# AdamCodd/local-hyperDB

Hardware: AMD Instinct MI355X
Metric: queries/sec, N=10M d=384 fp16 top-100 (single-query stream; p50 latency alongside) (higher is better)
Workload: dtype f16; 1 GPU; N=10000000 d=384 fp16 Q=1 cosine_similarity top-100, row-sharded x1; rows_per_gpu=10000000, accumulate=f32, exchange=none

## Files before the change

### local-hyperdb_amd/csrc/hdb_api.hip

```cpp
#include "hdb_common.h"
#include "hdb_quant.h"
#include "hdb_ws.h"
#include "hdb_plan.h"
#include "../../include/hyperdb_hip.h"
#include <string>
#include <cmath>
#include <cstring>
#include <cstdio>
#include <algorithm>
#include <vector>
#include <chrono>
#include <atomic>

static thread_local std::string g_err;
static int fail(int code, const std::string& msg) { g_err = msg; return code; }
#define HIP_TRY(expr)                                                                              \
    do {                                                                                           \
        hipError_t e_ = (expr);                                                                    \
        if (e_ != hipSuccess)                                                                      \
            return fail(HDB_ERR_HIP, std::string(#expr) + ": " + hipGetErrorString(e_));           \
    } while (0)
#define LAUNCH_TRY(expr)                                                                           \
    do {                                                                                           \
        int e_ = (expr);                                                                           \
// ... 638 lines not shown
    if (ix->n == 0) return HDB_OK;
    HIP_TRY(hipSetDevice(ix->device));
    hipStream_t st = (hipStream_t)stream;
    const int W = (ix->d + 31) / 32;
    ScoresWs w;
    int rc = ws_lay(ix, w, ix->d, W);
    if (rc) return rc;
    float* qinv = w.qinv; float* qsq = w.qsq; int* qnan = w.qnan; uint32_t* qbits = w.qbits; void* qc = w.qc;
    LAUNCH_TRY(hdb_launch_qprep(dev_q, 1, ix->d, ix->dtype == HDB_F64, qinv, qsq, qnan, nullptr, nullptr, st));
    if (is_bits_metric(metric)) {
        rc = ensure_bits(ix, st); if (rc) return rc;
        LAUNCH_TRY(hdb_launch_qsign(dev_q, 1, ix->d, ix->dtype == HDB_F64, W, qbits, st));
    }
    ScanArgs a; base_args(ix, a, dev_q, metric);
    if (metric == HDB_PEARSON) {
        rc = ensure_pscale(ix, st); if (rc) return rc;
        LAUNCH_TRY(hdb_launch_qcentre(dev_q, 1, ix->d, ix->dtype == HDB_F64, qc, qinv, st));
        a.Q = qc; a.metric = HDB_COSINE; a.inv_norm = ix->pscale;
    }
    a.mask = nullptr;
    a.raw = 1;
    a.scores = dev_out; a.ld = ix->n;
    QueryBufs qb{qinv, qsq, qbits, nullptr, nullptr};
    return run_scan(ix, a, 0, 1, qb, false, false, st);
}

struct TopkArgs { const void* Q; int32_t nq, k; int metric; int64_t* idx; float* score; int32_t* status; hipStream_t st; };
static TopkFacts topk_facts(const hdb_index* ix) {
    return {ix->n, ix->d, ix->dtype, ix->qmode, ix->qauto, ix->qauto_declined, ix->pnib != nullptr, ix->plane_declined,
            ix->mask != nullptr, ix->bias != nullptr, hdb_cu_count(), ix->subset_m};
}

static int quant_pitch(const hdb_index* ix) { return (int)align_up((size_t)ix->d, 16); }
static size_t quant_ws_bytes(const hdb_index* ix, int nq, uint32_t pl_cap, bool mflavour) {
    return ws_bytes_for<QuantWs>(nq, quant_pitch(ix), (int)ix->d, quant_ld_max(ix->n, ix->d), pl_cap, mflavour);
}
static int quant_ws_lay(hdb_index* ix, QuantWs& w, int nq, uint32_t pl_cap, bool mflavour) {
    return ws_lay(ix, w, nq, quant_pitch(ix), (int)ix->d, quant_ld_max(ix->n, ix->d), pl_cap, mflavour);
}
static size_t quant_batch_ws_bytes(const hdb_index* ix, int cq) {
    return ws_bytes_for<QuantBatchWs>(cq, quant_pitch(ix), (int)ix->d, quant_batch_sample(ix->n).ld_s, quant_batch_wld());
}
static int quant_batch_ws_lay(hdb_index* ix, QuantBatchWs& w, int cq) {
    return ws_lay(ix, w, cq, quant_pitch(ix), (int)ix->d, quant_batch_sample(ix->n).ld_s, quant_batch_wld());
}
static void quant_base_args(const hdb_index* ix, QuantArgs& a, const int8_t* qcodes, const float* qaux, const float* qinv, int metric, int nq) {
    memset(&a, 0, sizeof(a));
    a.codes = ix->qcodes; a.n = ix->n; a.d = ix->d; a.P = ix->qP; a.aux = ix->qaux; a.sqnorm = ix->sqnorm; a.inv_norm = ix->inv_norm;
    a.qcodes = qcodes; a.qaux = qaux; a.qinv = qinv; a.bias = ix->bias; a.mask = ix->mask; a.metric = metric; a.nq = nq;
    a.gamma = (float)quant_gamma(ix->d);
}
static int quant_query_prep(hdb_index* ix, const float* Q, int nq, const QuantWs& w, bool mflavour, int* stat, uint32_t* cnt_init,
                            uint32_t* pl_cnt, hipStream_t st) {
    if (mflavour) {
        LAUNCH_TRY(hdb_launch_quant_qprep_m(Q, nq, ix->d, ix->qP, w.qinv, w.qsq, w.qnan, w.q16, w.qscl, w.qcodes, w.qaux, stat, cnt_init, pl_cnt, st));
    } else {
        LAUNCH_TRY(hdb_launch_qprep(Q, nq, ix->d, false, w.qinv, w.qsq, w.qnan, nullptr, nullptr, st));
        LAUNCH_TRY(hdb_launch_quant_qprep(Q, nq, ix->d, ix->qP, w.qcodes, w.qaux, stat, pl_cnt, st));
    }
    return HDB_OK;
}

static int shadow_prepare(hdb_index* ix, const TopkPlan& p, int nq, hipStream_t st, bool* declined) {
    if (p.build_needed) {
        const size_t ws_need = p.path == HDB_PATH_QUANT ? quant_ws_bytes(ix, nq, 0, true) : quant_batch_ws_bytes(ix, p.cq_max);
        if (!quant_auto_build(ix, ws_need, st)) { *declined = true; return HDB_OK; }
    }
    if (p.plane_wanted && !ix->pnib) {
        const int rc = plane_rows(ix, 0, ix->n, st);
        if (rc) return rc;
        *declined = ix->pnib == nullptr;
    }
    return HDB_OK;
}

static int quant_topk(hdb_index* ix, const TopkArgs& c, const TopkPlan& p) {
    const void* dev_Q = c.Q; const int32_t nq = c.nq, k = c.k; const int metric = c.metric; hipStream_t st = c.st;
    int64_t* dev_idx = c.idx; float* dev_score = c.score; int32_t* dev_status = c.status;
    const uint32_t kk = p.kk; const bool mflavour = p.mflavour, use_pl = p.plane_wanted;
    const int64_t n = ix->n;
    const uint32_t m = 16;
    const QuantSample sp = p.qs;
    QuantWs w;
    int rc = quant_ws_lay(ix, w, nq, 0, mflavour);
    if (rc) return rc;
    uint32_t* qstat = reinterpret_cast<uint32_t*>(ix->qstat);
    uint32_t* pl_cnt = use_pl ? qstat + 1 : nullptr;
    const size_t crow = (size_t)nq * HDB_CAND_CAP;
    const int nsub = p.nsub;
    rc = quant_query_prep(ix, (const float*)dev_Q, nq, w, mflavour, ix->qstat, nsub ? w.cnt : nullptr, pl_cnt, st);
    if (rc) return rc;
    QuantArgs a; quant_base_args(ix, a, w.qcodes, w.qaux, w.qinv, metric, nq);
    a.ntiles = sp.s_tiles; a.tile_stride = sp.s_stride; a.scores = w.sbuf; a.ld = sp.ld_s;
    a.wmax = w.wmax; a.nsub = nsub; a.thr_out = w.thr;
    LAUNCH_TRY(hdb_launch_quant_scan(&a, 0, (int)ix->opt.max_blocks, st));
    if (!nsub) LAUNCH_TRY(hdb_launch_sample_thr(w.sbuf, sp.s_rows, sp.ld_s, nq, m, w.thr, w.cnt, nullptr, st));
    a.ntiles = (n + 15) / 16; a.tile_stride = 1; a.scores = nullptr; a.ld = 0;
    a.thr = w.thr; a.cnt = w.cnt; a.cand = w.cand; a.cap = HDB_CAND_CAP;
    const bool has_bias = ix->bias != nullptr || ix->mask != nullptr;
    if (mflavour) {
        a.V = (const char*)ix->V; a.row_bytes = ix->d * 2; a.G = w.G;
        a.ginv = metric == HDB_COSINE ? w.ginv : nullptr; a.gbias = has_bias ? w.gbias : nullptr;
    }
    prof_begin(ix, st);
    if (use_pl) {
        a.pl_nib = ix->pnib; a.pl_bit = ix->pbit; a.pl_rec = ix->prec; a.pl_units = ix->pU;
        a.pl_cnt = pl_cnt; a.pl_cap = p.pl_cap;
        LAUNCH_TRY(hdb_launch_quant_plane_scan(&a, 0, (int)ix->opt.max_blocks, st));
    } else {
        LAUNCH_TRY(hdb_launch_quant_scan(&a, 1, (int)ix->opt.max_blocks, st));
    }
    prof_end(ix, st);
    if (mflavour) {
        ScanArgs s; memset(&s, 0, sizeof(s));
        s.V = w.G; s.n = (int64_t)crow; s.d = ix->d; s.Q = dev_Q; s.metric = metric; s.inv_norm = w.ginv; s.qinv = w.qinv;
        s.bias = has_bias ? w.gbias : nullptr; s.mask = nullptr; s.nq = nq;
        s.tile_stride = 1; s.ntiles = (int64_t)crow / hdb_mfma_tile_rows(ix->dtype, ix->d); s.cap = HDB_CAND_CAP;
        s.scores = w.gsc; s.ld = (int64_t)crow;
        LAUNCH_TRY(hdb_launch_mfma_scan(&s, ix->dtype, 0, nq, w.q16, w.ginv, w.qsq, w.qscl, (int)ix->opt.max_blocks, (int)ix->opt.mfma_variant, st, nullptr));
    } else {
        LAUNCH_TRY(hdb_launch_quant_rescore(ix->V, ix->d, ix->dtype, (const float*)dev_Q, nq, metric, ix->inv_norm, w.qinv, ix->bias, ix->mask,
                                            w.cand, w.cnt, HDB_CAND_CAP, st));
    }
    LAUNCH_TRY(hdb_launch_quant_finalize(w.cand, w.cnt, HDB_CAND_CAP, nq, (uint32_t)k, kk, ix->row_base, dev_idx, dev_score, dev_status, w.qnan,
                                         w.qaux, w.thr, ix->qstat, mflavour ? w.cand : nullptr, w.gsc, (int64_t)crow, st));
    return HDB_OK;
}

extern "C" int hdb_debug_quant_bounds(hdb_index* ix, const float* dev_q, int metric, float* dev_hi, float* dev_hi5, void* stream) {
    if (!ix || !dev_q || !dev_hi || !dev_hi5) return fail(HDB_ERR_ARG, "hdb_debug_quant_bounds: null argument");
    if (metric != HDB_DOT && metric != HDB_COSINE) return fail(HDB_ERR_ARG, "hdb_debug_quant_bounds: dot or cosine");
    if (ix->qmode != HDB_QUANT_I8 || !ix->pnib || ix->n < 1) return fail(HDB_ERR_UNSUPPORTED, "hdb_debug_quant_bounds: the index has no 5-bit plane");
    HIP_TRY(hipSetDevice(ix->device));
    hipStream_t st = (hipStream_t)stream;
    QuantWs w;
    int rc = quant_ws_lay(ix, w, 1, 0, true);
    if (rc) return rc;
    rc = quant_query_prep(ix, dev_q, 1, w, ix->qauto, nullptr, nullptr, nullptr, st);
    if (rc) return rc;
    QuantArgs a; quant_base_args(ix, a, w.qcodes, w.qaux, w.qinv, metric, 1);
    a.ntiles = (ix->n + 15) / 16; a.tile_stride = 1;
    a.pl_nib = ix->pnib; a.pl_bit = ix->pbit; a.pl_rec = ix->prec; a.pl_units = ix->pU;
    a.dbg = dev_hi;
    LAUNCH_TRY(hdb_launch_quant_scan_one(&a, 2, (int)ix->opt.max_blocks, st));
    a.dbg = dev_hi5;
    LAUNCH_TRY(hdb_launch_quant_plane_scan(&a, 1, (int)ix->opt.max_blocks, st));
    return HDB_OK;
}

static int quant_batch_topk(hdb_index* ix, const TopkArgs& c, const TopkPlan& p) {
    const void* dev_Q = c.Q; const int32_t nq = c.nq, k = c.k; const int metric = c.metric; hipStream_t st = c.st;
    int64_t* dev_idx = c.idx; float* dev_score = c.score; int32_t* dev_status = c.status;
    const uint32_t kk = p.kk;
    const int64_t n = ix->n;
    const int P = ix->qP;
    const uint32_t m = HDB_QB_SAMPLE_M;
    const QuantSample sp = p.qs;
    const int64_t s_tiles = sp.s_tiles, s_stride = sp.s_stride, s_rows = sp.s_rows, ld_s = sp.ld_s;
    const int cq_max = p.cq_max;
    QuantBatchWs w;
    const int rc = quant_batch_ws_lay(ix, w, cq_max);
    if (rc) return rc;
    const int64_t wld = quant_batch_wld();
    float* const qinv = w.qinv; float* const qsq = w.qsq; int* const qnan = w.qnan; float* const qscl = w.qscl;
    int8_t* const qcodes = w.qcodes; float* const qaux = w.qaux; float* const thr = w.thr; uint32_t* const cnt = w.cnt;
    unsigned long long* const cand = w.cand; void* const q16 = w.q16; float* const wbuf = w.wbuf;
    for (int q0 = 0; q0 < nq; q0 += cq_max) {
        const int cq = std::min(cq_max, nq - q0);
        const float* Qc = (const float*)dev_Q + (size_t)q0 * ix->d;
// ... 673 lines not shown
```

### local-hyperdb_amd/csrc/hdb_caps.h

```cpp
#pragma once
#include "../../include/hyperdb_hip.h"

static inline int hdb_scan_auto_blocks(int dtype, int row_bytes, bool vec, bool wide_rows) {
    if (dtype == HDB_F8E4M3 && vec && (row_bytes == 256 || row_bytes == 384 || row_bytes == 512)) {
        const int b = 512 * 768 / row_bytes;
        return b < 1024 ? b : 1024;
    }
    return wide_rows ? 256 : 512;
}

#define HDB_KS_MAX_SLICES 8
struct KsGeom {
    int slices;
    int width[HDB_KS_MAX_SLICES];
    int off[HDB_KS_MAX_SLICES];
};
static inline KsGeom ks_list(int elem_bytes, int n0, int w0, int n1 = 0, int w1 = 0) {
    KsGeom g = {};
    int at = 0;
    for (int s = 0; s < n0 + n1 && s < HDB_KS_MAX_SLICES; ++s) {
        g.width[s] = s < n0 ? w0 : w1; g.off[s] = at * elem_bytes;
        at += g.width[s];
    }
    g.slices = n0 + n1;
// ... 127 lines not shown
static inline int hdb_mfma_fused_blocks(int64_t ntiles, int cus, int max_blocks) {
    int blocks = (int)(ntiles < cus ? ntiles : cus);
    if (max_blocks > 0 && max_blocks < blocks) blocks = max_blocks;
    if (blocks > HDB_FUSED_MAX_WG) blocks = HDB_FUSED_MAX_WG;
    if (blocks < 1) blocks = 1;
    return blocks;
}

#ifndef HDB_BITS_THREADS
#define HDB_BITS_THREADS 1024
#endif
#define HDB_BITS_MAXW 512
static inline int hdb_bits_fused_supported(int metric, int nq, int W, uint32_t kk) {
    return (metric == HDB_HAMMING || metric == HDB_JACCARD) && nq >= 1 && nq <= 4 && W <= HDB_BITS_MAXW && kk <= 128;
}
static inline int hdb_bits_fused_blocks(int64_t ntiles, int cus, int max_blocks) {
    int blocks = cus;
    const int64_t items = ntiles * 4;
    if ((int64_t)blocks * HDB_BITS_THREADS > items) blocks = (int)((items + HDB_BITS_THREADS - 1) / HDB_BITS_THREADS);
    if (max_blocks > 0 && max_blocks < blocks) blocks = max_blocks;
    if (blocks < 1) blocks = 1;
    return blocks;
}
static inline bool hdb_bits_fused_local(int blocks, uint32_t kk) { return (int64_t)blocks >= 2 * (int64_t)kk; }

static inline int hdb_l1_tile_supported(int dtype, int d) {
    if (dtype == HDB_F16) return d == 128 || d == 256 || d == 384 || d == 512 || d == 640 || d == 768;
    if (dtype == HDB_F32) return d == 128 || d == 256 || d == 384 || d == 512 || d == 768;
    return 0;
}

static inline int hdb_quant_scan_blocks(int64_t ntiles, int max_blocks) { return hdb_grid_for(ntiles, 4, max_blocks > 0 ? max_blocks : 1024); }
static inline int hdb_quant_plane_units(int P) { return (P + 31) / 32; }

static inline int hdb_qb_supported(int d) { return d == 128 || d == 256 || d == 384 || d == 512; }
static inline void qb_shape(int nq, int& wq, int& nqt) {
    const int tq = (nq + 15) / 16;
    wq = tq <= 4 ? 1 : tq <= 8 ? 2 : 4;
    nqt = (tq + wq - 1) / wq;
}
static inline int hdb_qb_scan_blocks(int64_t ntiles, int nq, int cus, int max_blocks) {
    int wq, nqt; qb_shape(nq, wq, nqt);
    const int64_t lim = max_blocks > 0 ? max_blocks : 2 * (int64_t)cus;
    return hdb_grid_for(ntiles, 4 / wq, (int)(lim < 512 ? lim : 512));
}
static inline int64_t hdb_qb_slots(int blocks, int nq) { int wq, nqt; qb_shape(nq, wq, nqt); return (int64_t)blocks * (4 / wq) * 4; }
```

### local-hyperdb_amd/csrc/hdb_common.h

```cpp
#pragma once
#include <hip/hip_runtime.h>
#include <hip/hip_fp16.h>
#include <stdint.h>

#define HDB_WAVE 64

__host__ __device__ __forceinline__ int hdb_elem_bytes(int dtype) {
    return dtype == 0 ? 2 : dtype == 1 ? 4 : dtype == 2 ? 8 : dtype == 3 ? 2 : dtype == 5 ? 1 : 0;
}
struct hdb_bf16 { unsigned short bits; };
__host__ __device__ __forceinline__ float hdb_bf16_to_f(hdb_bf16 v) {
    const unsigned int u = (unsigned int)v.bits << 16;
    return __builtin_bit_cast(float, u);
}

struct hdb_f8 { unsigned char bits; };
__host__ __device__ __forceinline__ float hdb_f8_to_f(hdb_f8 v) {
    const unsigned int b = v.bits, mag = b & 0x7Fu, sgn = (b & 0x80u) << 24;
    float r;
    if (mag == 0x7Fu) r = __builtin_bit_cast(float, 0x7FC00000u);
    else if (mag < 8u) r = (float)mag * 0.001953125f;
    else r = __builtin_bit_cast(float, mag << 20) * __builtin_bit_cast(float, 0x7B800000u);
    return __builtin_bit_cast(float, __builtin_bit_cast(unsigned int, r) | sgn);
}
// ... 82 lines not shown
typedef unsigned int hdb_u32x4 __attribute__((ext_vector_type(4)));
template <bool NT>
__device__ __forceinline__ uint4 hdb_bits_load(const uint32_t* bits, int64_t i, int w, int W) {
    const hdb_u32x4* p = reinterpret_cast<const hdb_u32x4*>(bits + (((i >> 6) * W + w) << 8) + 4 * (i & 63));
    const hdb_u32x4 v = NT ? __builtin_nontemporal_load(p) : *p;
    return make_uint4(v.x, v.y, v.z, v.w);
}

#define HDB_CNT_STRIDE 32

struct BitsArgs {
    const uint32_t* bits; int64_t npad; int32_t W;
    int64_t n; int32_t d;
    const float* Qraw; int32_t nq;
    int64_t ntiles, s_tiles, s_stride;
    const float* bias; const uint8_t* mask;
    uint32_t epoch, timeout_ticks;
    uint32_t* ctl;
    unsigned long long* cand; uint32_t cap, k, kk;
    int64_t row_base;
    int64_t* idx_out; float* score_out; int32_t* status;
    int32_t local;
};

__device__ __forceinline__ float hdb_q16_scale(float amax) {
    if (!(amax > 0.f) || !(amax < INFINITY)) return 1.f;
    int ex = 0;
    (void)frexpf(amax, &ex);
    int sh = 15 - ex;
    sh = sh < -100 ? -100 : (sh > 100 ? 100 : sh);
    return ldexpf(1.f, sh);
}

__device__ __forceinline__ int64_t hdb_tile_index(int64_t t, int64_t stride) {
    if (stride == 1) return t;
    const uint32_t h = (uint32_t)t * 2654435761u;
    return t * stride + (int64_t)((h >> 8) % (uint32_t)stride);
}

__device__ __forceinline__ uint32_t hdb_f2key(float f) {
    uint32_t u = __float_as_uint(f);
    return u ^ ((u >> 31) ? 0xFFFFFFFFu : 0x80000000u);
}
__device__ __forceinline__ float hdb_key2f(uint32_t k) {
    uint32_t u = k ^ ((k >> 31) ? 0x80000000u : 0xFFFFFFFFu);
    return __uint_as_float(u);
}
__device__ __forceinline__ unsigned long long hdb_pack(float s, uint32_t row) {
    return ((unsigned long long)hdb_f2key(s) << 32) | (unsigned long long)(0xFFFFFFFFu - row);
}
__device__ __forceinline__ float hdb_canon(float s) {
    if (s != s) s = -INFINITY;
    return s + 0.0f;
}

template <int CTRL>
__device__ __forceinline__ float hdb_dpp(float x) {
    return __int_as_float(__builtin_amdgcn_update_dpp(0, __float_as_int(x), CTRL, 0xF, 0xF, false));
}
template <int CTRL>
__device__ __forceinline__ double hdb_dpp(double x) {
    const long long b = __double_as_longlong(x);
    const int lo = __builtin_amdgcn_update_dpp(0, (int)(b & 0xFFFFFFFFll), CTRL, 0xF, 0xF, false);
    const int hi = __builtin_amdgcn_update_dpp(0, (int)(b >> 32), CTRL, 0xF, 0xF, false);
    return __longlong_as_double(((long long)hi << 32) | (unsigned int)lo);
}
#define HDB_DPP_MIRROR 0x140
// ... 56 lines not shown
```

### local-hyperdb_amd/csrc/hdb_quant.h

```cpp
#pragma once
#include <stdint.h>

#define HDB_QROW_S 0
#define HDB_QROW_E 1
#define HDB_QROW_T 2
#define HDB_QQ_S 0
#define HDB_QQ_N 1
#define HDB_QQ_D 2
#define HDB_QQ_SQ 3
#define HDB_QQ_BAD 4
#define HDB_QQ_CN 5
#define HDB_QQ_CS 6
#define HDB_QQ_WORDS 8

struct QuantArgs {
    const int8_t* codes;
    int64_t n;
    int32_t d;
    int32_t P;
    const float* aux;
    const float* sqnorm;
    const float* inv_norm;
    const int8_t* qcodes;
    const float* qaux;
    const float* qinv;
    const float* bias;
    const uint8_t* mask;
    int32_t metric;
    int32_t nq;
    float gamma;
    int64_t ntiles;
    int64_t tile_stride;
    float* scores; int64_t ld;
    const float* thr; uint32_t* cnt; unsigned long long* cand; uint32_t cap;
    uint32_t* wmax; int32_t nsub; float* thr_out;
    const char* V; int32_t row_bytes; char* G; float* ginv; float* gbias;
    const uint8_t* pl_nib; const uint32_t* pl_bit; const float* pl_rec; int32_t pl_units;
    uint32_t* pl_cnt; uint32_t pl_cap;
    float* dbg;
};
#define HDB_QUANT_NSUB_MAX 4096
```

### local-hyperdb_amd/csrc/hdb_quant.hip

```cpp
#include "hdb_common.h"
#include "hdb_quant.h"
#include "hdb_finalize.h"
#include "../../include/hyperdb_hip.h"

__device__ __forceinline__ float hq_up(double x) {
    x = x * (1.0 + 0x1p-40);
    float f = (float)x;
    if ((double)f < x) f = nextafterf(f, INFINITY);
    return f;
}

__device__ __forceinline__ float hq_f(__half v) { return __half2float(v); }
__device__ __forceinline__ float hq_f(float v) { return v; }

template <typename T> struct HqElem;
template <> struct HqElem<__half> { static constexpr int EPC = 8; };
template <> struct HqElem<float> { static constexpr int EPC = 4; };

__device__ __forceinline__ void hq_unpack(const uint4& raw, float (&x)[8], __half*) {
    const __half2* h = reinterpret_cast<const __half2*>(&raw);
#pragma unroll
    for (int i = 0; i < 4; ++i) { float2 f = __half22float2(h[i]); x[2 * i] = f.x; x[2 * i + 1] = f.y; }
}
__device__ __forceinline__ void hq_unpack(const uint4& raw, float (&x)[4], float*) {
// ... 203 lines not shown
    switch (ctrl_id) {
    case 0: return __builtin_amdgcn_update_dpp(0, x, HDB_DPP_MIRROR, 0xF, 0xF, false);
    case 1: return __builtin_amdgcn_update_dpp(0, x, HDB_DPP_HALF_MIRROR, 0xF, 0xF, false);
    case 2: return __builtin_amdgcn_update_dpp(0, x, HDB_DPP_XOR2, 0xF, 0xF, false);
    default: return __builtin_amdgcn_update_dpp(0, x, HDB_DPP_XOR1, 0xF, 0xF, false);
    }
}
__device__ __forceinline__ int hq_rows4_sum(int a0, int a1, int a2, int a3, int l16) {
    const bool b3 = (l16 & 8) != 0, b2 = (l16 & 4) != 0;
    const int v01 = (b3 ? a1 : a0) + hq_dpp_i(b3 ? a0 : a1, 0);
    const int v23 = (b3 ? a3 : a2) + hq_dpp_i(b3 ? a2 : a3, 0);
    int w = (b2 ? v23 : v01) + hq_dpp_i(b2 ? v01 : v23, 1);
    w += hq_dpp_i(w, 2);
    w += hq_dpp_i(w, 3);
    return w;
}

template <int NQ>
__device__ __forceinline__ void hq_fold_thr(const QuantArgs& a, float (&q_thr)[NQ]) {
    __shared__ uint32_t s_top[4 * 16];
    __shared__ float s_thr[NQ];
    const int ln = threadIdx.x & 63, wv = threadIdx.x >> 6;
    for (int q = 0; q < NQ; ++q) {
        uint32_t c[HDB_QUANT_NSUB_MAX / 256];
#pragma unroll
        for (int j = 0; j < HDB_QUANT_NSUB_MAX / 256; ++j) {
            const int e = (int)threadIdx.x + 256 * j;
            c[j] = e < a.nsub ? a.wmax[(int64_t)q * a.nsub + e] : 0u;
        }
        for (int r = 0; r < 16; ++r) {
            uint32_t lm = 0u;
#pragma unroll
            for (int j = 0; j < HDB_QUANT_NSUB_MAX / 256; ++j) lm = max(lm, c[j]);
            uint32_t wm = lm;
#pragma unroll
            for (int o = 32; o > 0; o >>= 1) wm = max(wm, (uint32_t)__shfl_xor((int)wm, o, 64));
            const unsigned long long who = __ballot(lm == wm);
            if (ln == (int)__ffsll((long long)who) - 1) {
                bool gone = false;
#pragma unroll
                for (int j = 0; j < HDB_QUANT_NSUB_MAX / 256; ++j)
                    if (!gone && c[j] == wm) { c[j] = 0u; gone = true; }
            }
            if (ln == 0) s_top[wv * 16 + r] = wm;
        }
        __syncthreads();
        if (wv == 0) {
            uint32_t v = s_top[ln];
            uint32_t kth = 0u;
            for (int r = 0; r < 16; ++r) {
                uint32_t wm = v;
#pragma unroll
                for (int o = 32; o > 0; o >>= 1) wm = max(wm, (uint32_t)__shfl_xor((int)wm, o, 64));
                const unsigned long long who = __ballot(v == wm);
                if (ln == (int)__ffsll((long long)who) - 1) v = 0u;
                kth = wm;
            }
            if (ln == 0) {
                const float t = kth == 0u ? -INFINITY : hdb_key2f(kth);
                s_thr[q] = t;
                if (blockIdx.x == 0) a.thr_out[q] = t;
            }
        }
        __syncthreads();
    }
#pragma unroll
    for (int q = 0; q < NQ; ++q) q_thr[q] = s_thr[q];
}

template <int NQ>
struct HqQuery {
    float s[NQ], n[NQ], d[NQ], sq[NQ], inv[NQ];
    bool bad[NQ];
};
template <int NQ>
__device__ __forceinline__ void hq_query_load(const QuantArgs& a, HqQuery<NQ>& qc) {
#pragma unroll
    for (int q = 0; q < NQ; ++q) {
        const float* o = a.qaux + (int64_t)q * HDB_QQ_WORDS;
        qc.s[q] = o[HDB_QQ_S]; qc.n[q] = o[HDB_QQ_N]; qc.d[q] = o[HDB_QQ_D]; qc.sq[q] = o[HDB_QQ_SQ]; qc.bad[q] = o[HDB_QQ_BAD] != 0.f;
        qc.inv[q] = a.metric == HDB_COSINE ? a.qinv[q] : 1.f;
    }
}

template <int NQ, int NJ, int G, typename Sink>
__device__ __forceinline__ bool hq_rows4_bounds(const QuantArgs& a, const int4* qs, const HqQuery<NQ>& qc, const int64_t (&rr)[4], int l16,
// ... 147 lines not shown
    extern __shared__ __attribute__((aligned(16))) char smem[];
    int4* qs = reinterpret_cast<int4*>(smem);
    __shared__ HqStage stage;
    const int nch = a.P >> 4;
    if (MODE == 1 && threadIdx.x < 4) stage.cnt[threadIdx.x] = 0u;
    for (int i = threadIdx.x; i < NQ * nch; i += 256) qs[i] = reinterpret_cast<const int4*>(a.qcodes)[i];
    HqQuery<NQ> qc;
    hq_query_load<NQ>(a, qc);
    float q_thr[NQ];
#pragma unroll
    for (int q = 0; q < NQ; ++q) q_thr[q] = (MODE == 1 && a.nsub == 0) ? a.thr[q] : 0.f;
    __syncthreads();
    if (MODE == 1 && a.nsub > 0) hq_fold_thr<NQ>(a, q_thr);

    const int lane = threadIdx.x & 63, wave = threadIdx.x >> 6;
    const int g = lane >> 4, l16 = lane & 15;
    uint32_t wbest[NQ];
#pragma unroll
    for (int q = 0; q < NQ; ++q) wbest[q] = 0u;

    const int64_t ntiles = a.ntiles;
    for (int64_t t = (int64_t)blockIdx.x * 4 + wave; t < ntiles; t += (int64_t)gridDim.x * 4) {
        const int64_t r0 = hdb_tile_index(t, a.tile_stride) * 16 + 4 * g;
        const int64_t rr[4] = {r0, r0 + 1, r0 + 2, r0 + 3};
        const int u_own = hdb_owned_row(l16);
        const int64_t row = r0 + u_own;
        const int64_t out_i = t * 16 + 4 * g + u_own;
        const bool live = hq_rows4_bounds<NQ, NJ, (NJ > 0 ? NJ : 2)>(a, qs, qc, rr, l16, row, [&](int q, float lo, float hi, bool masked) {
            if (MODE == 2) {
                a.dbg[row] = hi;
            } else if (MODE == 0) {
                if (a.nsub > 0) wbest[q] = max(wbest[q], hdb_f2key(lo));
                else a.scores[(int64_t)q * a.ld + out_i] = lo;
            } else if (!masked && !qc.bad[q] && hi >= q_thr[q]) {
                hq_emit(stage, q, hi, row);
            }
        });
        if (MODE == 0 && a.nsub == 0 && !live && (l16 & 3) == 0)
#pragma unroll
            for (int q = 0; q < NQ; ++q) a.scores[(int64_t)q * a.ld + out_i] = -INFINITY;
    }
    if (MODE == 0 && a.nsub > 0) {
#pragma unroll
        for (int q = 0; q < NQ; ++q) {
            uint32_t wm = wbest[q];
#pragma unroll
            for (int o = 32; o > 0; o >>= 1) wm = max(wm, (uint32_t)__shfl_xor((int)wm, o, 64));
            if (lane == 0) a.wmax[(int64_t)q * a.nsub + blockIdx.x * 4 + wave] = wm;
        }
    }
    if (MODE == 1) hq_stage_flush<NQ>(stage);
}

__global__ __launch_bounds__(256) void hdb_quant_plane_rows_kernel(const int8_t* codes, const float* aux, int64_t row0, int64_t m, int d, int P,
                                                                   int U, uint8_t* nib, uint32_t* bitw, float* rec) {
    const int lane = threadIdx.x & 63, g = lane >> 4, l16 = lane & 15;
    const int64_t wave = ((int64_t)blockIdx.x * 256 + threadIdx.x) >> 6;
    const int64_t nwaves = ((int64_t)gridDim.x * 256) >> 6;
    for (int64_t base = wave * 4; base < m; base += nwaves * 4) {
        const int64_t r = row0 + base + g;
        const bool valid = base + g < m;
        int ss = 0;
        if (valid && l16 < U) {
            const int8_t* src = codes + r * (int64_t)P + 32 * l16;
            uint4 raw[2];
            raw[0] = *reinterpret_cast<const uint4*>(src);
            raw[1] = (32 * l16 + 16 < P) ? *reinterpret_cast<const uint4*>(src + 16) : make_uint4(0u, 0u, 0u, 0u);
            const uint32_t* cw = reinterpret_cast<const uint32_t*>(raw);
            uint32_t nw[4] = {0u, 0u, 0u, 0u}, bw = 0u;
#pragma unroll
            for (int w = 0; w < 8; ++w) {
#pragma unroll
                for (int b = 0; b < 4; ++b) {
// ... 50 lines not shown
        for (int j = 0; j < J; ++j) {
            const int f = lane + 64 * j;
            const int unit = f < npieces ? f % U : 0;
            const int4 x = qs[2 * unit], y = qs[2 * unit + 1];
            qw[j][0] = x.x; qw[j][1] = x.y; qw[j][2] = x.z; qw[j][3] = x.w;
            qw[j][4] = y.x; qw[j][5] = y.y; qw[j][6] = y.z; qw[j][7] = y.w;
        }
    };
    load_qw();
    const float absmin = 0x1p-100f * (float)(a.d + 8);
    typedef unsigned int u32x4 __attribute__((ext_vector_type(4)));
    typedef float f32x4 __attribute__((ext_vector_type(4)));
    const int64_t ntiles = a.ntiles;
    const int et = lane >> 4, er = lane & 15;
    int qn = 0;
    uint32_t nsurv = 0u;
    auto drain = [&](int base, int m) {
        const QuantArgs& a = hq_args_in_memory();
        HqQuery<1> qc;
        qc.s[0] = q_s; qc.n[0] = q_n; qc.d[0] = q_d; qc.sq[0] = 0.f; qc.inv[0] = q_inv; qc.bad[0] = q_bad;
        int ln = lane;
        asm volatile("" : "+v"(ln));
        const int g = ln >> 4, l16 = ln & 15;
        int64_t rr[4];
#pragma unroll
        for (int u = 0; u < 4; ++u) rr[u] = 4 * g + u < m ? (int64_t)queue[wave][base + 4 * g + u] : a.n;
        const int own = 4 * g + hdb_owned_row(l16);
        const int64_t row = own < m ? (int64_t)queue[wave][base + own] : a.n;
        hq_rows4_bounds<1, 0, 1>(a, qs, qc, rr, l16, row, [&](int, float, float hi, bool masked) {
            if (!masked && !q_bad && hi >= q_thr) hq_emit(stage, 0, hi, row);
        });
    };

    for (int64_t t = ((int64_t)blockIdx.x * 4 + wave) * 2; t < ntiles; t += (int64_t)gridDim.x * 8) {
        u32x4 nv[2][J];
        uint32_t bv[2][J];
        int ln = lane;
        asm volatile("" : "+v"(ln));
#pragma unroll
        for (int tt = 0; tt < 2; ++tt) {
            const int pieces_left = (int)min((int64_t)16, max((int64_t)0, a.n - (t + tt) * 16)) * U;
            const uint8_t* nb = a.pl_nib + (t + tt) * (int64_t)npieces * 16;
            const uint32_t* bb = a.pl_bit + (t + tt) * (int64_t)npieces;
#pragma unroll
            for (int j = 0; j < J; ++j) {
                if (ln < pieces_left - 64 * j) {
                    nv[tt][j] = __builtin_nontemporal_load(reinterpret_cast<const u32x4*>(nb + (uint32_t)ln * 16u) + 64 * j);
                    bv[tt][j] = __builtin_nontemporal_load(bb + (uint32_t)ln + 64 * j);
                } else {
                    nv[tt][j] = u32x4{0u, 0u, 0u, 0u};
                    bv[tt][j] = 0u;
                }
            }
        }
        const int64_t row = (t + et) * 16 + er;
        const bool rvalid = lane < 32 && t + et < ntiles && row < a.n;
        f32x4 rc = f32x4{0.f, 0.f, 0.f, 0.f};
        float invn = 1.f, bias = 0.f;
        bool masked = false;
        if (rvalid) {
            rc = __builtin_nontemporal_load(reinterpret_cast<const f32x4*>(a.pl_rec) + row);
            if (cosine) invn = a.inv_norm[row];
            if (a.bias) bias = a.bias[row];
            if (a.mask) masked = !a.mask[row];
        }
        __builtin_amdgcn_sched_barrier(0);
#pragma unroll
        for (int tt = 0; tt < 2; ++tt) {
#pragma unroll
            for (int j = 0; j < J; ++j) {
                const uint32_t bw = bv[tt][j];
                const uint32_t w4[4] = {nv[tt][j].x, nv[tt][j].y, nv[tt][j].z, nv[tt][j].w};
                int s = 0;
#pragma unroll
                for (int i = 0; i < 4; ++i) {
                    const uint32_t lo = ((w4[i] << 1) & 0x1E1E1E1Eu) | ((bw >> (2 * i)) & 0x01010101u);
                    const uint32_t hi = ((w4[i] >> 3) & 0x1E1E1E1Eu) | ((bw >> (2 * i + 1)) & 0x01010101u);
                    s = __builtin_amdgcn_sdot4((int)lo, qw[j][2 * i], s, false);
                    s = __builtin_amdgcn_sdot4((int)hi, qw[j][2 * i + 1], s, false);
                }
                part[wave][tt][lane + 64 * j] = s;
            }
        }
        __builtin_amdgcn_fence(__ATOMIC_RELEASE, "wavefront");
        __builtin_amdgcn_wave_barrier();
        __builtin_amdgcn_fence(__ATOMIC_ACQUIRE, "wavefront");
        int S = 0;
        if (lane < 32)
            for (int i = 0; i < U; ++i) S += part[wave][et][er * U + i];
// ... 15 lines not shown
            const float Bmax = c0 + Amax * 0x1p-10f + absmin;
            const float Mx = Amax + Bmax;
            float X = (A5 + B5) + (Mx * 0x1p-18f + 1e-30f);
            float mM = Mx * (1.f + 0x1p-17f);
            if (cosine) { X = X * invn * q_inv; mM = mM * invn * q_inv; }
            const float Z = mM + fabsf(bias);
            float h = X;
            if (a.bias) h += bias;
            hi5 = h + (Z * 0x1p-18f + 4e-30f);
            if (hi5 != hi5) hi5 = INFINITY;
        }
        if (DBG) {
            if (rvalid) a.dbg[row] = hi5;
            continue;
        }
        const bool keep = !dead && !(hi5 < q_thr);
        const unsigned long long km = __ballot(keep);
        if (km == 0ull) continue;
        if (keep) queue[wave][qn + __popcll(km & ((1ull << lane) - 1ull))] = (uint32_t)row;
        const int nk = __popcll(km);
        qn += nk; nsurv += (uint32_t)nk;
        __builtin_amdgcn_fence(__ATOMIC_RELEASE, "wavefront");
        __builtin_amdgcn_wave_barrier();
        __builtin_amdgcn_fence(__ATOMIC_ACQUIRE, "wavefront");
        if (qn >= 16) {
            do { qn -= 16; drain(qn, 16); } while (qn >= 16);
            __builtin_amdgcn_fence(__ATOMIC_RELEASE, "wavefront");
            __builtin_amdgcn_wave_barrier();
            asm volatile("" ::: "memory");
            load_qw();
        }
    }
    if (!DBG) {
        if (qn > 0) drain(0, qn);
        if (lane == 0 && nsurv != 0u) atomicAdd(&surv_cnt, nsurv);
        hq_stage_flush<1>(stage);
        if (threadIdx.x == 0 && surv_cnt != 0u) {
            const QuantArgs& a = hq_args_in_memory();
            const uint32_t before = atomicAdd(&a.pl_cnt[0], surv_cnt);
            if (before <= a.pl_cap && before + surv_cnt > a.pl_cap) atomicAdd(&a.pl_cnt[1], 1u);
        }
    }
}

struct RescoreArgs {
    const void* V; int32_t d; int32_t row_bytes; int32_t nchunks;
    const float* Q;
    int32_t metric;
    const float* inv_norm; const float* qinv; const float* bias; const uint8_t* mask;
    unsigned long long* cand; const uint32_t* cnt; uint32_t cap;
};

template <typename T, int ACC, bool VEC>
__global__ __launch_bounds__(256) void hdb_quant_rescore_kernel(RescoreArgs a) {
    using Acc = float;
    constexpr int EPC = HqElem<T>::EPC;
    const int q = blockIdx.y;
    const int lane = threadIdx.x & 63, wave = threadIdx.x >> 6;
    const int g = lane >> 4, l16 = lane & 15;
    const uint32_t total = min(a.cnt[q * HDB_CNT_STRIDE], a.cap);
    const float* qv = a.Q + (int64_t)q * a.d;
    const char* Vb = reinterpret_cast<const char*>(a.V);
    const T* Vt = reinterpret_cast<const T*>(a.V);
    for (uint32_t base = ((uint32_t)blockIdx.x * 4 + wave) * 4; base < total; base += gridDim.x * 16) {
        const uint32_t i = base + g;
        const bool valid = i < total;
// ... 123 lines not shown
}
static bool hq_copy_args_ok(const QuantArgs& a) {
    return !a.G || (a.V && a.row_bytes > 0 && a.row_bytes % 16 == 0 && (reinterpret_cast<uintptr_t>(a.V) & 15) == 0 && (reinterpret_cast<uintptr_t>(a.G) & 15) == 0);
}
extern "C" int hdb_launch_quant_scan(const QuantArgs* args, int mode, int max_blocks, void* stream) {
    const QuantArgs& a = *args;
    if (a.nq < 1 || a.nq > 4 || (a.P & 15) != 0) return (int)hipErrorInvalidValue;
    const size_t lds = (size_t)a.nq * a.P;
    const int blocks = hdb_quant_scan_blocks(a.ntiles, max_blocks);
    if (a.nsub != 0 && (a.nsub > HDB_QUANT_NSUB_MAX || !a.wmax || (mode == 0 ? a.nsub != 4 * blocks : !a.thr_out))) return (int)hipErrorInvalidValue;
    if (mode == 0) hq_launch_scan_mode<0>(a, blocks, lds, (hipStream_t)stream);
    else {
        if (!hq_copy_args_ok(a)) return (int)hipErrorInvalidValue;
        hq_launch_scan_mode<1>(a, blocks, lds, (hipStream_t)stream);
    }
    return (int)hipGetLastError();
}

extern "C" int hdb_launch_quant_plane_rows(const int8_t* codes, const float* aux, int64_t row0, int64_t m, int d, int P, uint8_t* nib,
                                           uint32_t* bitw, float* rec, void* stream) {
    if (m <= 0) return 0;
    const int U = hdb_quant_plane_units(P);
    if (U > 16 || (P & 15) != 0) return (int)hipErrorInvalidValue;
    hipLaunchKernelGGL(hdb_quant_plane_rows_kernel, dim3(hdb_grid_for(m, 16, 8192)), dim3(256), 0, (hipStream_t)stream, codes, aux, row0, m, d,
                       P, U, nib, bitw, rec);
    return (int)hipGetLastError();
}
extern "C" int hdb_launch_quant_plane_scan(const QuantArgs* args, int dbg, int max_blocks, void* stream) {
    const QuantArgs& a = *args;
    const int U = a.pl_units;
    if (a.nq != 1 || U < 1 || U > 16 || U != hdb_quant_plane_units(a.P) || (a.metric != HDB_DOT && a.metric != HDB_COSINE)) return (int)hipErrorInvalidValue;
    if (!dbg && a.nsub != 0 && (a.nsub > HDB_QUANT_NSUB_MAX || !a.wmax || !a.thr_out)) return (int)hipErrorInvalidValue;
    if (!dbg && (!a.cnt || !a.cand || !a.pl_cnt || !hq_copy_args_ok(a))) return (int)hipErrorInvalidValue;
    const size_t lds = (size_t)U * 32;
    const int blocks = hdb_grid_for((a.ntiles + 1) / 2, 4, max_blocks > 0 ? max_blocks : 1024);
    hipStream_t st = (hipStream_t)stream;
    const int J = (U + 3) / 4;
#define HQ_PLANE(J_) do { if (dbg) hipLaunchKernelGGL((hdb_quant_plane_scan_kernel<J_, true>), dim3(blocks), dim3(256), lds, st, a); \
                          else hipLaunchKernelGGL((hdb_quant_plane_scan_kernel<J_, false>), dim3(blocks), dim3(256), lds, st, a); } while (0)
    if (J == 1) HQ_PLANE(1); else if (J == 2) HQ_PLANE(2); else if (J == 3) HQ_PLANE(3); else HQ_PLANE(4);
#undef HQ_PLANE
    return (int)hipGetLastError();
}
extern "C" int hdb_launch_quant_scan_one(const QuantArgs* args, int mode, int max_blocks, void* stream) {
    const QuantArgs& a = *args;
    if (a.nq != 1 || (a.P & 15) != 0 || a.nsub != 0 || mode != 2 || !a.dbg) return (int)hipErrorInvalidValue;
    const size_t lds = (size_t)a.P;
    const int blocks = hdb_quant_scan_blocks(a.ntiles, max_blocks);
    const int nj = ((a.P >> 4) + 15) >> 4;
    hipStream_t st = (hipStream_t)stream;
#define HQ_ONE(NJ_) hipLaunchKernelGGL((hdb_quant_scan_kernel<2, 1, NJ_>), dim3(blocks), dim3(256), lds, st, a)
    if (nj == 1) HQ_ONE(1); else if (nj == 2) HQ_ONE(2); else if (nj == 3) HQ_ONE(3); else HQ_ONE(0);
#undef HQ_ONE
    return (int)hipGetLastError();
}

extern "C" int hdb_launch_quant_rescore(const void* V, int d, int dtype, const float* Q, int nq, int metric, const float* inv_norm,
                                        const float* qinv, const float* bias, const uint8_t* mask, unsigned long long* cand,
                                        const uint32_t* cnt, uint32_t cap, void* stream) {
    hipStream_t st = (hipStream_t)stream;
    RescoreArgs a;
    a.V = V; a.d = d; a.Q = Q; a.metric = metric; a.inv_norm = inv_norm; a.qinv = qinv; a.bias = bias; a.mask = mask;
    a.cand = cand; a.cnt = cnt; a.cap = cap;
    const int elem = hdb_elem_bytes(dtype);
    a.row_bytes = d * elem;
    a.nchunks = a.row_bytes / 16;
    const bool vec = (a.row_bytes % 16 == 0) && ((reinterpret_cast<uintptr_t>(V) & 15) == 0) && ((size_t)d * 4 <= 60 * 1024);
    const bool euc = metric == HDB_EUCLIDEAN;
// ... 26 lines not shown
```

Measured before the change: 1917 queries/s.

## Reuse sampled-tile hi bounds to skip re-scanning sampled tiles in plane scan

The sampling pass over strided tiles now also writes each row's upper-bound score into a workspace list. The plane scan then walks only the tiles that were not sampled, using a skip-position iterator, and afterwards filters the sampled rows by comparing the stored bounds against the threshold, with no second full-precision pass over those tiles. The goal is to avoid rescanning the sampled fraction of the database, at the cost of extra workspace, extra index arithmetic per tile, and a serial filter loop at the end of each wave. Wave max reductions are also switched to a DPP helper.

```diff
diff --git a/local-hyperdb_amd/csrc/hdb_api.hip b/local-hyperdb_amd/csrc/hdb_api.hip
--- a/local-hyperdb_amd/csrc/hdb_api.hip
+++ b/local-hyperdb_amd/csrc/hdb_api.hip
@@ -694,6 +694,9 @@
 }
 
 static int quant_pitch(const hdb_index* ix) { return (int)align_up((size_t)ix->d, 16); }
+static uint32_t quant_hi_cap(const hdb_index* ix, int nq) {
+    return nq == 1 && plane_possible((int)ix->d) ? (uint32_t)quant_ld_max(ix->n, ix->d) : 0u;
+}
 static size_t quant_ws_bytes(const hdb_index* ix, int nq, uint32_t pl_cap, bool mflavour) {
     return ws_bytes_for<QuantWs>(nq, quant_pitch(ix), (int)ix->d, quant_ld_max(ix->n, ix->d), pl_cap, mflavour);
 }
@@ -725,7 +728,7 @@
 
 static int shadow_prepare(hdb_index* ix, const TopkPlan& p, int nq, hipStream_t st, bool* declined) {
     if (p.build_needed) {
-        const size_t ws_need = p.path == HDB_PATH_QUANT ? quant_ws_bytes(ix, nq, 0, true) : quant_batch_ws_bytes(ix, p.cq_max);
+        const size_t ws_need = p.path == HDB_PATH_QUANT ? quant_ws_bytes(ix, nq, quant_hi_cap(ix, nq), true) : quant_batch_ws_bytes(ix, p.cq_max);
         if (!quant_auto_build(ix, ws_need, st)) { *declined = true; return HDB_OK; }
     }
     if (p.plane_wanted && !ix->pnib) {
@@ -744,7 +747,7 @@
     const uint32_t m = 16;
     const QuantSample sp = p.qs;
     QuantWs w;
-    int rc = quant_ws_lay(ix, w, nq, 0, mflavour);
+    int rc = quant_ws_lay(ix, w, nq, quant_hi_cap(ix, nq), mflavour);
     if (rc) return rc;
     uint32_t* qstat = reinterpret_cast<uint32_t*>(ix->qstat);
     uint32_t* pl_cnt = use_pl ? qstat + 1 : nullptr;
@@ -755,6 +758,8 @@
     QuantArgs a; quant_base_args(ix, a, w.qcodes, w.qaux, w.qinv, metric, nq);
     a.ntiles = sp.s_tiles; a.tile_stride = sp.s_stride; a.scores = w.sbuf; a.ld = sp.ld_s;
     a.wmax = w.wmax; a.nsub = nsub; a.thr_out = w.thr;
+    a.pl_hi = use_pl ? reinterpret_cast<float*>(w.pl_list) : nullptr;
+    if (use_pl && (!a.pl_hi || sp.s_rows > (int64_t)quant_hi_cap(ix, nq))) return fail(HDB_ERR_ARG, "quant_topk: no list for the sampled rows");
     LAUNCH_TRY(hdb_launch_quant_scan(&a, 0, (int)ix->opt.max_blocks, st));
     if (!nsub) LAUNCH_TRY(hdb_launch_sample_thr(w.sbuf, sp.s_rows, sp.ld_s, nq, m, w.thr, w.cnt, nullptr, st));
     a.ntiles = (n + 15) / 16; a.tile_stride = 1; a.scores = nullptr; a.ld = 0;
@@ -768,6 +773,7 @@
     if (use_pl) {
         a.pl_nib = ix->pnib; a.pl_bit = ix->pbit; a.pl_rec = ix->prec; a.pl_units = ix->pU;
         a.pl_cnt = pl_cnt; a.pl_cap = p.pl_cap;
+        a.pl_s_tiles = (uint32_t)sp.s_tiles; a.pl_s_stride = (uint32_t)sp.s_stride;
         LAUNCH_TRY(hdb_launch_quant_plane_scan(&a, 0, (int)ix->opt.max_blocks, st));
     } else {
         LAUNCH_TRY(hdb_launch_quant_scan(&a, 1, (int)ix->opt.max_blocks, st));
@@ -796,7 +802,7 @@
     HIP_TRY(hipSetDevice(ix->device));
     hipStream_t st = (hipStream_t)stream;
     QuantWs w;
-    int rc = quant_ws_lay(ix, w, 1, 0, true);
+    int rc = quant_ws_lay(ix, w, 1, quant_hi_cap(ix, 1), true);
     if (rc) return rc;
     rc = quant_query_prep(ix, dev_q, 1, w, ix->qauto, nullptr, nullptr, nullptr, st);
     if (rc) return rc;
diff --git a/local-hyperdb_amd/csrc/hdb_caps.h b/local-hyperdb_amd/csrc/hdb_caps.h
--- a/local-hyperdb_amd/csrc/hdb_caps.h
+++ b/local-hyperdb_amd/csrc/hdb_caps.h
@@ -183,6 +183,35 @@
 
 static inline int hdb_quant_scan_blocks(int64_t ntiles, int max_blocks) { return hdb_grid_for(ntiles, 4, max_blocks > 0 ? max_blocks : 1024); }
 static inline int hdb_quant_plane_units(int P) { return (P + 31) / 32; }
+struct HdbSkipPos { uint32_t w, o; };
+struct HdbSkipStep { uint32_t dw, dn, step; };
+__host__ __device__ __forceinline__ uint32_t hdb_plane_skip_count(uint32_t ntiles, uint32_t s_tiles) { return ntiles - s_tiles; }
+__host__ __device__ __forceinline__ HdbSkipStep hdb_plane_skip_step(uint32_t step, uint32_t stride) {
+    const uint32_t m = stride - 1u;
+    HdbSkipStep s;
+    s.dw = m ? step / m : 0u; s.dn = m ? step % m : 0u; s.step = step;
+    return s;
+}
+__host__ __device__ __forceinline__ HdbSkipPos hdb_plane_skip_start(uint32_t tp, uint32_t s_tiles, uint32_t stride) {
+    const uint32_t m = stride - 1u;
+    HdbSkipPos p;
+    const uint32_t w = m ? tp / m : s_tiles;
+    if (w < s_tiles) { p.w = w; p.o = tp - w * m; }
+    else { p.w = s_tiles; p.o = tp - s_tiles * m; }
+    return p;
+}
+__host__ __device__ __forceinline__ void hdb_plane_skip_advance(HdbSkipPos& p, const HdbSkipStep& s, uint32_t s_tiles, uint32_t stride) {
+    if (p.w >= s_tiles) { p.o += s.step; return; }
+    const uint32_t m = stride - 1u;
+    p.w += s.dw; p.o += s.dn;
+    if (p.o >= m) { p.o -= m; ++p.w; }
+    if (p.w >= s_tiles) { p.o += (p.w - s_tiles) * m; p.w = s_tiles; }
+}
+__host__ __device__ __forceinline__ int64_t hdb_plane_skip_tile(const HdbSkipPos& p, uint32_t s_tiles, uint32_t stride) {
+    if (p.w >= s_tiles) return (int64_t)s_tiles * stride + p.o;
+    const uint32_t jit = (uint32_t)(hdb_tile_index((int64_t)p.w, (int64_t)stride) - (int64_t)p.w * stride);
+    return (int64_t)p.w * stride + p.o + (p.o >= jit ? 1u : 0u);
+}
 
 static inline int hdb_qb_supported(int d) { return d == 128 || d == 256 || d == 384 || d == 512; }
 static inline void qb_shape(int nq, int& wq, int& nqt) {
diff --git a/local-hyperdb_amd/csrc/hdb_common.h b/local-hyperdb_amd/csrc/hdb_common.h
--- a/local-hyperdb_amd/csrc/hdb_common.h
+++ b/local-hyperdb_amd/csrc/hdb_common.h
@@ -138,7 +138,7 @@
     return ldexpf(1.f, sh);
 }
 
-__device__ __forceinline__ int64_t hdb_tile_index(int64_t t, int64_t stride) {
+__host__ __device__ __forceinline__ int64_t hdb_tile_index(int64_t t, int64_t stride) {
     if (stride == 1) return t;
     const uint32_t h = (uint32_t)t * 2654435761u;
     return t * stride + (int64_t)((h >> 8) % (uint32_t)stride);
diff --git a/local-hyperdb_amd/csrc/hdb_quant.h b/local-hyperdb_amd/csrc/hdb_quant.h
--- a/local-hyperdb_amd/csrc/hdb_quant.h
+++ b/local-hyperdb_amd/csrc/hdb_quant.h
@@ -37,6 +37,7 @@
     const char* V; int32_t row_bytes; char* G; float* ginv; float* gbias;
     const uint8_t* pl_nib; const uint32_t* pl_bit; const float* pl_rec; int32_t pl_units;
     uint32_t* pl_cnt; uint32_t pl_cap;
+    float* pl_hi; uint32_t pl_s_tiles; uint32_t pl_s_stride;
     float* dbg;
 };
 #define HDB_QUANT_NSUB_MAX 4096
diff --git a/local-hyperdb_amd/csrc/hdb_quant.hip b/local-hyperdb_amd/csrc/hdb_quant.hip
--- a/local-hyperdb_amd/csrc/hdb_quant.hip
+++ b/local-hyperdb_amd/csrc/hdb_quant.hip
@@ -259,9 +259,7 @@
             uint32_t lm = 0u;
 #pragma unroll
             for (int j = 0; j < HDB_QUANT_NSUB_MAX / 256; ++j) lm = max(lm, c[j]);
-            uint32_t wm = lm;
-#pragma unroll
-            for (int o = 32; o > 0; o >>= 1) wm = max(wm, (uint32_t)__shfl_xor((int)wm, o, 64));
+            const uint32_t wm = hdb_wave_max_dpp(lm);
             const unsigned long long who = __ballot(lm == wm);
             if (ln == (int)__ffsll((long long)who) - 1) {
                 bool gone = false;
@@ -276,9 +274,7 @@
             uint32_t v = s_top[ln];
             uint32_t kth = 0u;
             for (int r = 0; r < 16; ++r) {
-                uint32_t wm = v;
-#pragma unroll
-                for (int o = 32; o > 0; o >>= 1) wm = max(wm, (uint32_t)__shfl_xor((int)wm, o, 64));
+                const uint32_t wm = hdb_wave_max_dpp(v);
                 const unsigned long long who = __ballot(v == wm);
                 if (ln == (int)__ffsll((long long)who) - 1) v = 0u;
                 kth = wm;
@@ -492,6 +488,7 @@
             } else if (MODE == 0) {
                 if (a.nsub > 0) wbest[q] = max(wbest[q], hdb_f2key(lo));
                 else a.scores[(int64_t)q * a.ld + out_i] = lo;
+                if (NQ == 1 && a.pl_hi) a.pl_hi[out_i] = hi;
             } else if (!masked && !qc.bad[q] && hi >= q_thr[q]) {
                 hq_emit(stage, q, hi, row);
             }
@@ -499,6 +496,7 @@
         if (MODE == 0 && a.nsub == 0 && !live && (l16 & 3) == 0)
 #pragma unroll
             for (int q = 0; q < NQ; ++q) a.scores[(int64_t)q * a.ld + out_i] = -INFINITY;
+        if (MODE == 0 && NQ == 1 && a.pl_hi && !live && (l16 & 3) == 0) a.pl_hi[out_i] = -INFINITY;
     }
     if (MODE == 0 && a.nsub > 0) {
 #pragma unroll
@@ -615,16 +613,28 @@
         });
     };
 
-    for (int64_t t = ((int64_t)blockIdx.x * 4 + wave) * 2; t < ntiles; t += (int64_t)gridDim.x * 8) {
+    const uint32_t s_tiles = DBG ? 0u : a.pl_s_tiles, s_stride = DBG ? 1u : a.pl_s_stride;
+    const uint32_t nwalk = hdb_plane_skip_count((uint32_t)ntiles, s_tiles);
+    const uint32_t tp0 = ((uint32_t)blockIdx.x * 4u + (uint32_t)wave) * 2u;
+    const HdbSkipStep sk_step = hdb_plane_skip_step((uint32_t)gridDim.x * 8u, s_stride), sk_next = {0u, 1u, 1u};
+    HdbSkipPos pos = hdb_plane_skip_start(tp0 < nwalk ? tp0 : 0u, s_tiles, s_stride);
+    for (uint32_t tp = tp0; tp < nwalk; tp += (uint32_t)gridDim.x * 8u, hdb_plane_skip_advance(pos, sk_step, s_tiles, s_stride)) {
+        int64_t tl[2];
+        {
+            HdbSkipPos p1 = pos;
+            hdb_plane_skip_advance(p1, sk_next, s_tiles, s_stride);
+            tl[0] = hdb_plane_skip_tile(pos, s_tiles, s_stride);
+            tl[1] = tp + 1u < nwalk ? hdb_plane_skip_tile(p1, s_tiles, s_stride) : ntiles;
+        }
         u32x4 nv[2][J];
         uint32_t bv[2][J];
         int ln = lane;
         asm volatile("" : "+v"(ln));
 #pragma unroll
         for (int tt = 0; tt < 2; ++tt) {
-            const int pieces_left = (int)min((int64_t)16, max((int64_t)0, a.n - (t + tt) * 16)) * U;
-            const uint8_t* nb = a.pl_nib + (t + tt) * (int64_t)npieces * 16;
-            const uint32_t* bb = a.pl_bit + (t + tt) * (int64_t)npieces;
+            const int pieces_left = (int)min((int64_t)16, max((int64_t)0, a.n - tl[tt] * 16)) * U;
+            const uint8_t* nb = a.pl_nib + tl[tt] * (int64_t)npieces * 16;
+            const uint32_t* bb = a.pl_bit + tl[tt] * (int64_t)npieces;
 #pragma unroll
             for (int j = 0; j < J; ++j) {
                 if (ln < pieces_left - 64 * j) {
@@ -636,8 +646,8 @@
                 }
             }
         }
-        const int64_t row = (t + et) * 16 + er;
-        const bool rvalid = lane < 32 && t + et < ntiles && row < a.n;
+        const int64_t row = (et ? tl[1] : tl[0]) * 16 + er;
+        const bool rvalid = lane < 32 && row < a.n;
         f32x4 rc = f32x4{0.f, 0.f, 0.f, 0.f};
         float invn = 1.f, bias = 0.f;
         bool masked = false;
@@ -719,6 +729,36 @@
         }
     }
     if (!DBG) {
+        if (s_tiles != 0u) {
+            const QuantArgs& am = hq_args_in_memory();
+            const uint32_t nslots = s_tiles * 16u, dslot = (uint32_t)gridDim.x * 256u;
+            uint32_t cbase = ((uint32_t)blockIdx.x * 4u + (uint32_t)wave) * 64u;
+            float hnext = cbase + lane < nslots ? am.pl_hi[cbase + lane] : 0.f;
+#pragma unroll 1
+            for (; cbase < nslots; cbase += dslot) {
+                const uint32_t slot = cbase + lane;
+                const float hi = hnext;
+                hnext = slot + dslot < nslots ? am.pl_hi[slot + dslot] : 0.f;
+                const int64_t row = hdb_tile_index((int64_t)(slot >> 4), (int64_t)s_stride) * 16 + (slot & 15u);
+                bool keep = slot < nslots && !q_bad && !(hi < q_thr);
+                if (keep && am.mask) keep = am.mask[row] != 0;
+                const unsigned long long km = __ballot(keep);
+#pragma unroll 1
+                for (int h = 0; h < 2; ++h) {
+                    const uint32_t kh = (uint32_t)(km >> (32 * h));
+                    if (kh == 0u) continue;
+                    if (keep && (lane >> 5) == h) queue[wave][qn + __popc(kh & ((1u << (lane & 31)) - 1u))] = (uint32_t)row;
+                    const int nk = __popc(kh);
+                    qn += nk; nsurv += (uint32_t)nk;
+                    __builtin_amdgcn_fence(__ATOMIC_RELEASE, "wavefront");
+                    __builtin_amdgcn_wave_barrier();
+                    __builtin_amdgcn_fence(__ATOMIC_ACQUIRE, "wavefront");
+                    while (qn >= 16) { qn -= 16; drain(qn, 16); }
+                    __builtin_amdgcn_fence(__ATOMIC_RELEASE, "wavefront");
+                    __builtin_amdgcn_wave_barrier();
+                }
+            }
+        }
         if (qn > 0) drain(0, qn);
         if (lane == 0 && nsurv != 0u) atomicAdd(&surv_cnt, nsurv);
         hq_stage_flush<1>(stage);
@@ -908,8 +948,11 @@
     if (a.nq != 1 || U < 1 || U > 16 || U != hdb_quant_plane_units(a.P) || (a.metric != HDB_DOT && a.metric != HDB_COSINE)) return (int)hipErrorInvalidValue;
     if (!dbg && a.nsub != 0 && (a.nsub > HDB_QUANT_NSUB_MAX || !a.wmax || !a.thr_out)) return (int)hipErrorInvalidValue;
     if (!dbg && (!a.cnt || !a.cand || !a.pl_cnt || !hq_copy_args_ok(a))) return (int)hipErrorInvalidValue;
+    if (a.ntiles < 0 || a.ntiles > 0x10000000) return (int)hipErrorInvalidValue;
+    if (!dbg && a.pl_s_tiles != 0u && (!a.pl_hi || a.pl_s_stride < 1u || (uint64_t)a.pl_s_tiles * a.pl_s_stride > (uint64_t)a.ntiles)) return (int)hipErrorInvalidValue;
     const size_t lds = (size_t)U * 32;
-    const int blocks = hdb_grid_for((a.ntiles + 1) / 2, 4, max_blocks > 0 ? max_blocks : 1024);
+    const int64_t nwalk = a.ntiles - (dbg ? 0 : (int64_t)a.pl_s_tiles);
+    const int blocks = hdb_grid_for((nwalk + 1) / 2, 4, max_blocks > 0 ? max_blocks : 1024);
     hipStream_t st = (hipStream_t)stream;
     const int J = (U + 3) / 4;
 #define HQ_PLANE(J_) do { if (dbg) hipLaunchKernelGGL((hdb_quant_plane_scan_kernel<J_, true>), dim3(blocks), dim3(256), lds, st, a); \
```

After: 1960 queries/s, median of 6. 1.02x the previous value.
